# gnosisguild/stylus-zkvm-verifiers

Measured on AMD Instinct MI355X. Metric: Groth16 proofs verified/sec (BN254), higher is better.
Workload: dtype u32

## Files before the change

stylus_zkvm_verifiers_amd/build.py:

```python
import concurrent.futures as cf
import glob
import os
import subprocess
import sys

HERE = os.path.dirname(os.path.abspath(__file__))
CSRC = os.path.join(HERE, 'csrc')
BUILD = os.path.join(CSRC, 'build')
LIB = os.path.join(HERE, 'libzkv_mi355x.so')
UNITS = ['k_setup', 'k_gt', 'k_prep', 'k_msm', 'k_pair', 'k_wide', 'k_precompile', 'k_wire', 'k_mixed', 'k_diag', 'k_plonk', 'k_plonk_keys', 'k_plonk_set', 'k_pset_agg', 'k_agg', 'k_gset', 'k_gset_pair', 'k_gset_agg', 'k_gset_agg_pair', 'k_gateway', 'k_gateway_keys', 'k_risc0_router', 'k_setincl', 'k_rzrouter_set', 'k_wire_rzset', 'k_selftest', 'k_selftest_pair', 'zkv_capi']
FLAGS = ['--offload-arch=gfx950', '-O3', '-std=c++17', '-fPIC', '-fvisibility=hidden', '-DZKV_FP_MUL_NOINLINE',
         '-Rpass-analysis=kernel-resource-usage']
UNIT_FLAGS = {}
COMPILE_TIMEOUT_S = 1500
EXTRA = os.environ.get('ZKV_EXTRA_FLAGS', '').split()


def _hipcc():
    for c in ('/opt/rocm/bin/hipcc', 'hipcc'):
        if os.path.sep not in c or os.path.exists(c):
            return c
    return 'hipcc'


def _deps_mtime():
    files = glob.glob(os.path.join(CSRC, '*.h')) + [os.path.join(HERE, '..', 'include', f) for f in ('zkv.h', 'zkv_groth16_set.h', 'zkv_sp1_gateway.h', 'zkv_sp1_gateway_wire.h', 'zkv_sp1_gateway_keys.h', 'zkv_plonk_keys.h', 'zkv_plonk_set.h', 'zkv_plonk_set_agg.h', 'zkv_diag_primitive.h', 'zkv_diag_prep.h', 'zkv_diag_gt.h', 'zkv_risc0_set_inclusion.h', 'zkv_risc0_router.h', 'zkv_risc0_router_wire.h', 'zkv_risc0_router_set.h', 'zkv_risc0_router_set_wire.h')]
    return max(os.path.getmtime(f) for f in files)


def _compile(unit, force, dep_m):
    src = os.path.join(CSRC, unit + '.hip')
    obj = os.path.join(BUILD, unit + '.o')
    log = os.path.join(BUILD, unit + '.log')
    if not force and os.path.exists(obj) and os.path.getmtime(obj) >= max(os.path.getmtime(src), dep_m):
        return unit, 'cached'
    cmd = [_hipcc()] + FLAGS + UNIT_FLAGS.get(unit, []) + EXTRA + ['-c', src, '-o', obj]
    with open(log, 'w') as lf:
        try:
            rc = subprocess.run(cmd, stdout=lf, stderr=subprocess.STDOUT, timeout=COMPILE_TIMEOUT_S, cwd=CSRC).returncode
        except subprocess.TimeoutExpired:
            rc = 124
    if rc != 0:
        tail = open(log).read()[-4000:]
        raise RuntimeError('hipcc failed for %s (rc=%d)\n%s' % (unit, rc, tail))
    return unit, 'built'


def build(force=False, verbose=True):
    os.makedirs(BUILD, exist_ok=True)
    dep_m = _deps_mtime()
    with cf.ThreadPoolExecutor(max_workers=min(7, os.cpu_count() or 4)) as ex:
        results = list(ex.map(lambda u: _compile(u, force, dep_m), UNITS))
    objs = [os.path.join(BUILD, u + '.o') for u in UNITS]
    need_link = force or not os.path.exists(LIB) or any(os.path.getmtime(o) > os.path.getmtime(LIB) for o in objs)
    if need_link:
        subprocess.check_call([_hipcc(), '--offload-arch=gfx950', '-shared', '-fPIC', '-o', LIB] + objs)
    if verbose:
        print('libzkv_mi355x.so:', ', '.join('%s=%s' % r for r in results), '(linked)' if need_link else '(up to date)')
    return LIB
# ... 27 lines not shown
```

stylus_zkvm_verifiers_amd/csrc/k_pair.hip:

```cpp
#define ZKV_PAIRED 1
#include "zkv_internal.h"
#include "zkv_agg.h"

namespace zkv {

#ifndef ZKV_PAIR_WAVES
#define ZKV_PAIR_WAVES 1
#endif
constexpr int PAIR_BLOCK = ZKV_BLOCK * ZKV_PAIR_WAVES;

__device__ __forceinline__ Fp2 ld_b(const Workspace& ws, int word0, size_t i) {
    Fp2 r; r.h = ws_ld(ws.prep, ws.cap, word0 + 8 * (int)(threadIdx.x & 1u), i);
    return r;
}

__global__ __launch_bounds__(ZKV_BLOCK, 2) void k_g2chk2(size_t n, Workspace ws, uint8_t* __restrict__ status) {
    size_t i = ((size_t)blockIdx.x * ZKV_BLOCK + threadIdx.x) >> 1;
    if (i >= n) return;
    uint32_t flags = ws.flags[i];
    if (!(flags & FL_ALIVE) || (flags & FL_B_INF)) return;
    Fp2 bx = ld_b(ws, 32, i), by = ld_b(ws, 48, i);
    bool ok = g2_in_subgroup(bx, by);
    if (!ok && !(threadIdx.x & 1u)) { ws.g2bad[i] = 1; status[i] = ST_VERIFICATION_FAILED; }
}

#if defined(ZKV_STAMPS)
__device__ unsigned long long* g_zkv_stamps = nullptr;
extern "C" __attribute__((visibility("default"))) int zkv_diag_set_stamps(void* dev_ptr) {
    return (int)hipMemcpyToSymbol(HIP_SYMBOL(g_zkv_stamps), &dev_ptr, sizeof(dev_ptr));
}
__device__ __forceinline__ void zkv_stamp(unsigned kernel, unsigned slot) {
    if ((threadIdx.x & 63u) != 0 || !g_zkv_stamps) return;
    unsigned long long* row = g_zkv_stamps + ((size_t)kernel * gridDim.x * (blockDim.x >> 6) + (size_t)blockIdx.x * (blockDim.x >> 6) + (threadIdx.x >> 6)) * 8;
    row[slot] = __builtin_amdgcn_s_memrealtime();
    row[4 + slot] = __builtin_amdgcn_s_memtime();
    if (slot == 0) { row[2] = __builtin_amdgcn_s_getreg((31 << 11) | 4); row[3] = __builtin_amdgcn_s_getreg((31 << 11) | 20); }
}
#define ZKV_STAMP(k, s) zkv_stamp(k, s)
#else
#define ZKV_STAMP(k, s) ((void)0)
#endif

__global__ __launch_bounds__(PAIR_BLOCK, 2) void k_miller2(size_t n, const VkTables* __restrict__ vk, const uint32_t* __restrict__ mconst, Workspace ws, uint8_t* __restrict__ status) {
    __shared__ uint32_t lds[(48 + 24) * PAIR_BLOCK];
    ZKV_STAMP(0, 0);
    size_t i = ((size_t)blockIdx.x * PAIR_BLOCK + threadIdx.x) >> 1;
    if (i >= n) return;
    uint32_t flags = ws.flags[i];
    if (!(flags & FL_ALIVE)) return;
    const uint32_t par = threadIdx.x & 1u;
    uint32_t* wl = lds + (threadIdx.x >> 6) * ((48 + 24) * ZKV_BLOCK) + (threadIdx.x & 63u);
    LRef fm = l_ref(wl);
    LRef tm = l_ref(wl + 48 * ZKV_BLOCK);
    SoaRef norm = {ws.norm, ws.cap, (uint32_t)i * 4u};
    SoaRef bsrc = {ws.prep + 32 * ws.cap, ws.cap, (uint32_t)(8 * par * ws.cap + i) * 4u};
    const uint32_t* start = mconst ? mconst + 96 : nullptr;
    if (!miller_loop_p(vk, flags, norm, bsrc, fm, tm, true, start)) {
        if (!par) { ws.g2bad[i] = 1; status[i] = ST_VERIFICATION_FAILED; }
        return;
    }
    MRef out = m_ref(ws.f + (size_t)(8 * par) * ws.cap + i, (uint32_t)ws.cap, 16);
    if (start) f12m_copy(out, fm);
    else {
        MRef ab = m_ref((uint32_t*)vk->f_alpha_beta + 8 * par, 1, 16);
        f12m_mul_body(out, fm, ab, false);
    }
    ZKV_STAMP(0, 1);
}

__global__ __launch_bounds__(PAIR_BLOCK, 2) void k_finalexp2(size_t n, GtTab gt, long long gt_rel, long long gt_crel, Workspace ws, uint8_t* __restrict__ status) {
    __shared__ uint32_t lds[54 * PAIR_BLOCK];
    ZKV_STAMP(1, 0);
    size_t i = ((size_t)blockIdx.x * PAIR_BLOCK + threadIdx.x) >> 1;
    if (i >= n) return;
    uint32_t flags = ws.flags[i];
    if (!(flags & FL_ALIVE) || ws.g2bad[i]) return;
    const uint32_t par = threadIdx.x & 1u;
    uint32_t* wl = lds + (threadIdx.x >> 6) * (54 * ZKV_BLOCK) + (threadIdx.x & 63u);
    L9Ref acc = l9_ref(wl);
    const GtRef g = {gt.tab != nullptr, (ptrdiff_t)gt_rel, ws.prep + 64 * ws.cap, gt.nw[0], gt.nw[1], gt.cache ? ws.gtag : nullptr, (ptrdiff_t)gt_crel};
    bool one = final_exp_prog_p(ws.f, ws.fe, ws.cap, (uint32_t)(8 * par * ws.cap + i) * 4u, acc, g);
    if (!par) status[i] = one ? ST_OK : ST_VERIFICATION_FAILED;
    ZKV_STAMP(1, 1);
}

ZKV_HD bool pair_all(bool mine) {
    uint32_t v = mine ? 0u : 1u;
    v |= zkv_partner_u32(v);
    return v == 0;
}
// ... 270 lines not shown
```

stylus_zkvm_verifiers_amd/csrc/k_selftest_pair.hip:

```cpp
#define ZKV_PAIRED 1
#define ZKV_SELFTEST_BODIES 1
#include "zkv_internal.h"
#include "zkv_selftest.h"

namespace zkv {

__global__ __launch_bounds__(64) void k_selftest_pair(int op, int in_w, int out_w, const uint32_t* __restrict__ in, uint32_t* __restrict__ out) {
    __shared__ uint32_t lds[(144 + 54) * 64];
    const size_t i = (size_t)blockIdx.x * 32 + (threadIdx.x >> 1);
    selftest_pair(op, in + i * (size_t)in_w, out + i * (size_t)out_w, lds + threadIdx.x);
}
template <int S>
__device__ __forceinline__ void selftest_wide_body(int op, int in_w, int out_w, const uint32_t* in, uint32_t* out, uint32_t* lds) {
    constexpr int GROUP = 16 * S;
    const uint32_t g = threadIdx.x / GROUP;
    WL w;
    w.q = (int)((threadIdx.x >> 1) & 7u);
    if (w.q >= 6) w.q -= 6;
    w.s = (int)((threadIdx.x % GROUP) >> 4);
    const size_t i = (size_t)blockIdx.x * (64 / GROUP) + g;
    selftest_wide<S>(op, in + i * (size_t)in_w, out + i * (size_t)out_w, lds + g * ST_WIDE_SLOT, w);
}
__global__ __launch_bounds__(64) void k_selftest_wide_s1(int op, int in_w, int out_w, const uint32_t* __restrict__ in, uint32_t* __restrict__ out) {
    __shared__ uint32_t lds[4 * ST_WIDE_SLOT];
    selftest_wide_body<1>(op, in_w, out_w, in, out, lds);
}
__global__ __launch_bounds__(64) void k_selftest_wide_s4(int op, int in_w, int out_w, const uint32_t* __restrict__ in, uint32_t* __restrict__ out) {
    __shared__ uint32_t lds[ST_WIDE_SLOT];
    selftest_wide_body<4>(op, in_w, out_w, in, out, lds);
}

void launch_selftest_pair(int mapping, int op, unsigned waves, const uint32_t* in, uint32_t* out, hipStream_t s) {
    int iw = 0, ow = 0;
    selftest_io(mapping, op, &iw, &ow);
    if (mapping == 1) hipLaunchKernelGGL(k_selftest_pair, dim3(waves), dim3(64), 0, s, op, iw, ow, in, out);
    else if (mapping == 2) hipLaunchKernelGGL(k_selftest_wide_s1, dim3(waves), dim3(64), 0, s, op, iw, ow, in, out);
    else hipLaunchKernelGGL(k_selftest_wide_s4, dim3(waves), dim3(64), 0, s, op, iw, ow, in, out);
}

}
```

stylus_zkvm_verifiers_amd/csrc/zkv_capi.hip:

```cpp
#include <hip/hip_runtime.h>
#include <condition_variable>
#include <functional>
#include <memory>
#include <mutex>
#include <new>
#include <math.h>
#include <stdio.h>
#include <stdlib.h>
#include <string.h>
#include <system_error>
#include <thread>
#include <utility>
#include <vector>

#include "../../include/zkv.h"
#include "../../include/zkv_groth16_set.h"
#include "../../include/zkv_sp1_gateway.h"
#include "../../include/zkv_sp1_gateway_wire.h"
#include "../../include/zkv_sp1_gateway_keys.h"
#include "../../include/zkv_plonk_keys.h"
#include "../../include/zkv_plonk_set.h"
#include "../../include/zkv_plonk_set_agg.h"
#include "../../include/zkv_diag_primitive.h"
#include "../../include/zkv_diag_prep.h"
#include "../../include/zkv_diag_gt.h"
#include "../../include/zkv_risc0_set_inclusion.h"
#include "../../include/zkv_risc0_router.h"
#include "../../include/zkv_risc0_router_wire.h"
#include "../../include/zkv_risc0_router_set.h"
#include "../../include/zkv_risc0_router_set_wire.h"
#include "zkv_host_abi.h"
#include "zkv_host_vk.h"
#include "zkv_internal.h"
#include "zkv_devmem.h"
#include "zkv_plonk.h"
#include "zkv_agg.h"
#include "zkv_gset_layout.h"
#include "zkv_selftest.h"
#include "zkv_setincl.h"
#include "zkv_rzrouter_prep.h"
#include "zkv_wire_rzrouter.h"
#include "zkv_rzrouter_set.h"
#include "zkv_wire_rzset.h"
#include <sys/random.h>

using namespace zkv;

#define ZKV_EXPORT extern "C" __attribute__((visibility("default")))

struct ChunkMem {
    DevBuf<uint32_t> ws_prep, ws_norm, ws_f, ws_fe, ws_flags, ws_g2bad;
    DevBuf<uint8_t> ws_gtag;
    Workspace ws = {nullptr, nullptr, nullptr, nullptr, nullptr, nullptr, 0};
    DevBuf<uint8_t> d_a, d_b, d_status, d_recv;
    DevBuf<uint64_t> d_off, d_pvoff;
    DevBuf<uint32_t> d_inst_idx;
// ... 3386 lines not shown
    if (shader_clock_ghz) *shader_clock_ghz = clk[1] ? 0.1 * (double)clk[0] / (double)clk[1] : 0.0;
    return ZKV_OK;
}
ZKV_EXPORT int zkv_diag_mulmod_rate(int device, int kind, int waves_per_simd, uint32_t iters, double* mulmods_per_s, double* shader_clock_ghz) {
    if (kind < 0 || kind > 4 || waves_per_simd < 1 || waves_per_simd > 8 || !iters || !mulmods_per_s) return ZKV_ERR_INVALID_ARG;
    return run_diag(device, false, kind, waves_per_simd, iters, mulmods_per_s, shader_clock_ghz);
}
ZKV_EXPORT int zkv_diag_issue_rate(int device, int kind, int waves_per_simd, uint32_t iters, double* lane_instr_per_s, double* shader_clock_ghz) {
    if (kind < 0 || kind > 2 || waves_per_simd < 1 || waves_per_simd > 8 || !iters || !lane_instr_per_s) return ZKV_ERR_INVALID_ARG;
    return run_diag(device, true, kind, waves_per_simd, iters, lane_instr_per_s, shader_clock_ghz);
}

ZKV_EXPORT int zkv_diag_primitive(int device, int mapping, int op, size_t n, const uint32_t* in, uint32_t* out) {
    int iw = 0, ow = 0;
    if (!selftest_io(mapping, op, &iw, &ow) || n == 0 || n > ZKV_DIAG_PRIMITIVE_MAX_CASES || !in || !out) return ZKV_ERR_INVALID_ARG;
    int nd = 0;
    if (hipGetDeviceCount(&nd) != hipSuccess || nd <= 0) { (void)hipGetLastError(); return ZKV_ERR_NO_DEVICE; }
    if (device < 0 || device >= nd || !device_is_gfx950(device)) return ZKV_ERR_NO_DEVICE;
    HIP_TRY(hipSetDevice(device));
    const size_t per = (size_t)selftest_cases_per_wave(mapping), waves = (n + per - 1) / per, padded = waves * per;
    DevBuf<uint32_t> d_in, d_out;
    if (d_in.alloc(padded * (size_t)iw * 4) || d_out.alloc(padded * (size_t)ow * 4)) return ZKV_ERR_OOM;
    bool ok = hipMemset(d_in, 0, padded * (size_t)iw * 4) == hipSuccess && hipMemcpy(d_in, in, n * (size_t)iw * 4, hipMemcpyHostToDevice) == hipSuccess;
    if (ok) {
        if (mapping == 0) launch_selftest_lane(op, (unsigned)waves, d_in, d_out, nullptr);
        else launch_selftest_pair(mapping, op, (unsigned)waves, d_in, d_out, nullptr);
        ok = hipGetLastError() == hipSuccess && hipDeviceSynchronize() == hipSuccess &&
             hipMemcpy(out, d_out, n * (size_t)ow * 4, hipMemcpyDeviceToHost) == hipSuccess;
    }
    if (!ok) { (void)hipGetLastError(); return ZKV_ERR_HIP; }
    return ZKV_OK;
}

static_assert(ZKV_DIAG_PREP_SIGNALS == MAX_VAR, "zkv_diag_prep.h documents MAX_VAR signal rows");
ZKV_EXPORT int zkv_diag_prep_signals(zkv_ctx* c, size_t n, uint32_t* signals, uint32_t* flags) {
    if (!c || !signals || !flags || n == 0) return ZKV_ERR_INVALID_ARG;
    if (is_sharded(c) || (c->vm != ZKV_VM_RISC0 && c->vm != ZKV_VM_SP1) || c->agg_on) return ZKV_ERR_INVALID_ARG;
    int nd = 0;
    if (hipGetDeviceCount(&nd) != hipSuccess || nd <= 0) { (void)hipGetLastError(); return ZKV_ERR_NO_DEVICE; }
    if (c->device < 0 || c->device >= nd || !device_is_gfx950(c->device)) return ZKV_ERR_NO_DEVICE;
    std::lock_guard<std::mutex> lk(c->mu);
    if (!c->dev_ready || !c->ws.prep || n > c->last_chunk_n || n > c->ws.cap) return ZKV_ERR_INVALID_ARG;
    HIP_TRY(hipSetDevice(c->device));
    HIP_TRY(hipDeviceSynchronize());
    const size_t rows = (size_t)8 * MAX_VAR;
    std::vector<uint32_t> t(rows * n);
    HIP_TRY(hipMemcpy2D(t.data(), 4 * n, c->ws.prep + (size_t)64 * c->ws.cap, 4 * c->ws.cap, 4 * n, rows, hipMemcpyDeviceToHost));
    HIP_TRY(hipMemcpy(flags, c->ws.flags, 4 * n, hipMemcpyDeviceToHost));
    for (size_t j = 0; j < n; j++)
        for (size_t r = 0; r < rows; r++) signals[j * rows + r] = t[r * n + j];
    return ZKV_OK;
}

ZKV_EXPORT int zkv_ctx_vm(const zkv_ctx* c) { return c ? c->vm : ZKV_ERR_INVALID_ARG; }
ZKV_EXPORT int zkv_ctx_set_lanes_per_proof(zkv_ctx* c, int lanes) {
    if (!c || (lanes != 0 && lanes != 2 && lanes != 16 && lanes != 64 && lanes != 128)) return ZKV_ERR_INVALID_ARG;
    if (is_sharded(c)) { for (auto* k : c->shards) { const int rc = zkv_ctx_set_lanes_per_proof(k, lanes); if (rc != ZKV_OK) return rc; } return ZKV_OK; }
    if (c->vm == ZKV_VM_MIXED) {
        for (auto* k : c->kid) { const int rc = zkv_ctx_set_lanes_per_proof(k, lanes); if (rc != ZKV_OK) return rc; }
    }
    if (c->vm == ZKV_VM_RISC0_SETINCL) { const int rc = zkv_ctx_set_lanes_per_proof(c->kid[0], lanes); if (rc != ZKV_OK) return rc; }
    if (c->vm == ZKV_VM_RISC0_ROUTER && c->kid[0]) { const int rc = zkv_ctx_set_lanes_per_proof(c->kid[0], lanes); if (rc != ZKV_OK) return rc; }
    for (auto* k : c->gw_route) { if (!k) continue; const int rc = zkv_ctx_set_lanes_per_proof(k, lanes); if (rc != ZKV_OK) return rc; }
    if (c->gw_group) { const int rc = zkv_ctx_set_lanes_per_proof(c->gw_group, lanes); if (rc != ZKV_OK) return rc; }
    std::lock_guard<std::mutex> lk(c->mu);
    c->lanes = lanes;
// ... 906 lines not shown
```

stylus_zkvm_verifiers_amd/csrc/zkv_internal.h:

```cpp
#pragma once
#include <hip/hip_runtime.h>
#include "zkv_verify.h"

namespace zkv {

constexpr int WS_PREP_WORDS = 64 + 8 * MAX_VAR;
constexpr int WS_NORM_WORDS = 48;
constexpr int WS_F_WORDS = 96;
constexpr int WS_FE_WORDS = 7 * 96;
struct Workspace {
    uint32_t* prep; uint32_t* norm; uint32_t* f; uint32_t* fe; uint32_t* flags;
    uint32_t* g2bad;
    size_t cap;
    uint8_t* gtag;
};

constexpr int ZKV_BLOCK = 64;

__device__ __forceinline__ Fp ws_ld(const uint32_t* base, size_t cap, int word0, size_t i) {
    Fp r;
#pragma unroll
    for (int k = 0; k < 8; k++) r.v[k] = base[(size_t)(word0 + k) * cap + i];
    return r;
}
// ... 212 lines not shown
void launch_gset_agg_fprod(size_t n, size_t n2, uint32_t sub, uint32_t g, const Workspace& ws, const uint32_t* agg, const Workspace& ws2, const uint32_t* psl,
                           hipStream_t s);
void launch_gset_agg_mark(size_t n, uint32_t sub, uint32_t g, const Workspace& ws, const uint32_t* agg, const uint8_t* status2, const uint32_t* psl,
                          uint8_t* status, unsigned long long* counters, hipStream_t s);

#ifndef ZKV_PLONK_PROOF_BYTES
#define ZKV_PLONK_PROOF_BYTES 868
#endif
struct PlonkKeyRaw; struct PlonkKey;
void launch_plonk_setup(const PlonkKeyRaw* d_raw, PlonkKey* d_key, hipStream_t s);
void launch_plonk_setup_keys(const PlonkKeyRaw* d_raw, PlonkKey* d_key, hipStream_t s);
void launch_plonk_prep(const PrepArgs& a, const PlonkKey* d_key, const Workspace& ws, hipStream_t s);
void launch_plonk_prep_keys(const PrepArgs& a, const PlonkKey* d_key, const Workspace& ws, hipStream_t s);
struct PsetChunk {
    size_t m, slot0;
    const uint32_t* idx; const uint32_t* skey;
    const PlonkKey* keys; const uint32_t* ok;
    const uint8_t* proofs; uint32_t proof_stride;
    const uint8_t* inputs; uint32_t input_stride;
    uint32_t* plonk_tab;
    uint8_t* status;
};
void launch_pset_setup(uint32_t n_keys, const PlonkKeyRaw* d_raw, PlonkKey* d_keys, const VkTables* d_tabs, uint32_t* d_ok, hipStream_t s);
void launch_pset_prep(const PsetChunk& c, const Workspace& ws, hipStream_t s);
void launch_pset_agg_reduce(size_t m, uint32_t sub, const Workspace& ws, const uint32_t* agg, const Workspace& ws2, uint8_t* status2, const uint32_t* psl,
                            bool park, hipStream_t s);
void launch_pset_agg_combine(size_t n2, uint32_t wide, const Workspace& ws2, uint8_t* status2, const uint32_t* psl, hipStream_t s);

int read_wait_faults(unsigned long long* out);
void launch_diag_mulmod(int kind, unsigned blocks, uint32_t iters, uint32_t* out, unsigned long long* clk, hipStream_t s);
void launch_diag_issue(int kind, unsigned blocks, uint32_t iters, uint32_t* out, unsigned long long* clk, hipStream_t s);
void launch_selftest_lane(int op, unsigned waves, const uint32_t* in, uint32_t* out, hipStream_t s);
void launch_selftest_pair(int mapping, int op, unsigned waves, const uint32_t* in, uint32_t* out, hipStream_t s);

struct AggTables; struct AggSeed;
void launch_setup_agg(const VkRaw* d_raw, const VkTables* d_tab, AggTables* d_agg, hipStream_t s);
void launch_agg_g1(size_t n, const VkTables* d_tab, const InstTab* inst_tab, const Workspace& ws, uint32_t* agg, const AggSeed& seed, bool sums, hipStream_t s);
void launch_agg_reduce(size_t n, uint32_t sub, bool sums, uint32_t g, const VkTables* d_tab, const Workspace& ws, const uint32_t* agg, const AggTables* tab,
                       const Workspace& ws2, uint8_t* status2, bool park, hipStream_t s);
void launch_agg_combine(size_t n64, size_t n2, uint32_t wide, const AggTables* tab, const Workspace& ws2, uint8_t* status2, hipStream_t s);
void launch_agg_miller(size_t n, uint32_t g, const VkTables* d_tab, const Workspace& ws, uint8_t* status, hipStream_t s);
void launch_agg_fprod(size_t n, size_t n2, uint32_t sub, uint32_t g, const Workspace& ws, const uint32_t* agg, const Workspace& ws2, hipStream_t s);
void launch_agg_mark(size_t n, uint32_t sub, uint32_t g, const Workspace& ws, const uint32_t* agg, const uint8_t* status2, uint8_t* status, unsigned long long* counters,
                     uint32_t* idx, hipStream_t s);
void launch_agg_gather(size_t n, const Workspace& ws, const uint32_t* agg, const unsigned long long* counters, const uint32_t* idx, const Workspace& ws3,
                       uint8_t* status3, hipStream_t s);
void launch_agg_plonk_g1(size_t n, const Workspace& ws, uint32_t* agg, const AggSeed& seed, hipStream_t s);
void launch_agg_plonk_norm(size_t n, const Workspace& ws, const uint32_t* agg, const unsigned long long* counters, const uint32_t* idx, const Workspace& ws3,
                           uint8_t* status3, hipStream_t s);
void launch_agg_scatter(size_t n, const unsigned long long* counters, const uint32_t* idx, const uint8_t* status3, uint8_t* status, hipStream_t s);

void launch_ecadd(size_t n, const uint8_t* in, uint8_t* out, uint8_t* ok, hipStream_t s);
void launch_ecmul(size_t n, const uint8_t* in, uint8_t* out, uint8_t* ok, hipStream_t s);
void launch_pairing(size_t n, uint32_t k, const uint8_t* in, const Workspace& ws, uint8_t* result, uint8_t* ok, hipStream_t s);
uint32_t pairing_group(uint32_t k);
void launch_pairing_w(size_t n, uint32_t k, const uint8_t* in, const Workspace& ws, uint8_t* result, uint8_t* ok, hipStream_t s);

}
```

stylus_zkvm_verifiers_amd/csrc/zkv_selftest.h:

```cpp
#pragma once
#include <stdint.h>

namespace zkv {

inline bool selftest_io(int mapping, int op, int* in_w, int* out_w) {
    static const int LANE[11][2] = {{24, 128}, {24, 16}, {16, 16}, {8, 8}, {32, 64}, {24, 40}, {8, 12}, {64, 72}, {32, 2}, {128, 248}, {112, 384}};
    static const int PAIR[10][2] = {{32, 80}, {162, 18}, {36, 18}, {240, 11 * 96}, {96, 2 * 96}, {32, 4}, {192, 6}, {80, 2}, {192, 816}, {32, 4}};
    static const int WIDE[4][2] = {{240, 8 * 96}, {96, 96}, {96, 16}, {288, 0}};
    const int* w = nullptr;
    if (mapping == 0 && op >= 0 && op < 11) w = LANE[op];
    else if (mapping == 1 && op >= 0 && op < 10) w = PAIR[op];
    else if ((mapping == 2 || mapping == 3) && op >= 0 && op < 4) w = WIDE[op];
    if (!w) return false;
    *in_w = w[0]; *out_w = (mapping == 3 && op == 2) ? 4 * w[1] : w[1];
    if (mapping >= 2 && op == 3) *out_w = 2 * (48 + 48 * 8 * (mapping == 3 ? 4 : 1)) + 5 * 96 + 48;
    return true;
}
inline int selftest_cases_per_wave(int mapping) { return mapping == 0 ? 64 : mapping == 1 ? 32 : mapping == 2 ? 4 : 1; }

}

#if defined(ZKV_SELFTEST_BODIES)
#if defined(ZKV_PAIRED)
#include "zkv_tower_wide.h"
// ... 217 lines not shown
                line_add(T, qx, qy, l0, l1, l3);
            }
            m_st_f2(tm, 0, T.x); m_st_f2(tm, 1, T.y); m_st_f2(tm, 2, T.z);
        };
        auto put = [&](uint32_t* o, const Fp2& l0, const Fp2& l1, const Fp2& l3) {
            for (int k = 0; k < 3; k++) st_st(o + 16 * k + 8 * par, m_ld_f2(tm, k).h);
            st_st(o + 48 + 8 * par, l0.h); st_st(o + 64 + 8 * par, l1.h); st_st(o + 80 + 8 * par, l3.h);
        };
        Fp2 l0, l1, l3, t0, t1, t3;
        load_t(); step(0, t0, t1, t3); put(out, t0, t1, t3);
        for (int kind = 1; kind <= 4; kind++) { load_t(); step(kind, l0, l1, l3); put(out + 96 * kind, l0, l1, l3); }
        f12m_copy(fm, m_ref((uint32_t*)in + 96 + 8 * par, 1, 16));
        {
            const Fp2 c3 = f2_mul_fp(t1, norm.fp(0)), c4 = f2_mul_fp(t3, norm.fp(8));
            f12m_mul_by_034_body(fm, t0, c3, c4);
        }
        f12m_copy(m_ref(out + 480 + 8 * par, 1, 16), fm);
        load_t(); step(0, l0, l1, l3); step(1, l0, l1, l3); step(0, l0, l1, l3);
        for (int k = 0; k < 3; k++) st_st(out + 576 + 16 * k + 8 * par, m_ld_f2(tm, k).h);
        load_t(); g2m_line_dbl(tm, &l0, &l1, &l3); put(out + 624, l0, l1, l3);
        const Fp2 qx = st_ldh(in + 48, par), qy = st_ldh(in + 64, par);
        load_t(); g2m_line_add(tm, &qx, &qy, &l0, &l1, &l3); put(out + 720, l0, l1, l3);
        break;
    }
    case 9: {
        const Fp2 qx = st_ldh(in, par), qy = st_ldh(in + 16, par);
        out[par] = g2_on_twist(qx, qy) ? 1u : 0u; out[2 + par] = g2_in_subgroup(qx, qy) ? 1u : 0u;
        break;
    }
    default: break;
    }
}

constexpr int ST_WIDE_SLOT = 96 + 48 + 13 * 16 + W_RED_WORDS;
template <int S> ZKV_HD int st_group_lane(WL w, uint32_t par) {
#if defined(__HIP_DEVICE_COMPILE__)
    (void)w; (void)par;
    return (int)(__builtin_amdgcn_mbcnt_hi(~0u, __builtin_amdgcn_mbcnt_lo(~0u, 0u)) & (uint32_t)(16 * S - 1));
#else
    return 16 * w.s + 2 * w.q + (int)par;
#endif
}
template <int S> ZKV_HD void selftest_wide(int op, const uint32_t* in, uint32_t* out, uint32_t* g, WL w) {
    const uint32_t par = zkv_parity();
    const int q = w.q;
    uint32_t* base = g + 8 * par;
    const MRef A = m_ref(base, 1, 16), B = m_ref(base + 96, 1, 16), D = m_ref(base + 192, 1, 16), red = m_ref(base + 288, 1, 16);
    const MRef ga = m_ref((uint32_t*)in + 8 * par, 1, 16), gb = m_ref((uint32_t*)in + 96 + 8 * par, 1, 16);
    auto put = [&](int k) { w12_copy(m_ref(out + 96 * k + 8 * par, 1, 16), D, q); };
    switch (op) {
    case 0: {
        const Fp2 c0 = st_ldh(in + 192, par), c3 = st_ldh(in + 208, par), c4 = st_ldh(in + 224, par);
        w12_copy(A, ga, q); w12_copy(B, gb, q);
        w12_copy(D, A, q); w12_mul<S>(D, D, B, w, false, red); put(0);
        w12_copy(D, A, q); w12_mul<S>(D, D, B, w, true, red); put(1);
        w12_copy(D, A, q); w12_sqr<S>(D, w, red); put(2);
        w12_copy(D, A, q); w12_mul_sparse<S>(D, &c0, &c3, &c4, w, false, red); put(3);
        w12_copy(D, A, q); w12_mul_sparse<S>(D, &c3, &c3, &c4, w, true, red); put(4);
        for (int k = 1; k <= 3; k++) { w12_frob(D, A, k, q); put(4 + k); }
        break;
    }
    case 1: {
        w12_copy(D, ga, q); w12_cyclo_sqr<S>(D, w, red); put(0);
        break;
    }
    case 2: {
// ... 50 lines not shown
```

stylus_zkvm_verifiers_amd/csrc/zkv_verify.h:

```cpp
#pragma once
#include "zkv_tower_mem.h"
#include "zkv_sha256.h"
#include "zkv_gt.h"

namespace zkv {

enum : uint8_t {
    ST_OK = 0, ST_VERIFICATION_FAILED = 1, ST_INVALID_INITIALIZATION = 2, ST_ALREADY_INITIALIZED = 3,
    ST_INVALID_PROOF_DATA = 4, ST_SELECTOR_MISMATCH = 5,
    ST_BAD_CALLDATA = 6
};
enum : uint32_t { FL_ALIVE = 1u, FL_A_INF = 2u, FL_B_INF = 4u, FL_C_INF = 8u, FL_L_INF = 16u };

constexpr int N_LINES = 88;
constexpr int MSM_MAX_WINDOWS = 32;
constexpr int MSM_DIGITS = 256;
constexpr int MAX_IC = 6;
constexpr int MAX_VAR = 5;

struct VkRaw {
    uint32_t alpha[2][8];
    uint32_t beta[4][8], gamma[4][8], delta[4][8];
    uint32_t ic[MAX_IC][2][8];
    uint32_t n_ic;
    uint32_t fixed_scalar[MAX_IC][8];
    uint32_t is_fixed[MAX_IC];
    uint32_t n_var;
    uint32_t var_ic[MAX_VAR];
    uint32_t var_windows[MAX_VAR];
};

struct VkTables {
    G1A base; uint32_t base_inf; uint32_t n_var; uint32_t var_windows[MAX_VAR];
    uint32_t vk_valid;
// ... 228 lines not shown
            }
            if (do_l) fixed_line_mul(fm, lines0[li], n.lxs, n.lys);
            if (do_c) fixed_line_mul(fm, lines1[li], n.cxs, n.cys);
            li++;
        }
    }
    Fp2 qx[2], qy[2];
    g2_frob_affine(qx[0], qy[0], bx, by);
    g2_frob2_affine(qx[1], qy[1], bx, by);
    qy[1] = f2_neg(qy[1]);
#pragma unroll 1
    for (int s = 0; s < 2; s++) {
        if (do_t) {
            g2m_line_add(tm, &qx[s], &qy[s], &l0, &l1, &l3);
            if (do_ab) var_line_mul(fm, l0, l1, l3, n.axs, n.ays);
        }
        if (do_l) fixed_line_mul(fm, lines0[li], n.lxs, n.lys);
        if (do_c) fixed_line_mul(fm, lines1[li], n.cxs, n.cys);
        li++;
    }
    return !(check_b && do_t) || miller_point_closes(tm, bx, by);
}

#if defined(ZKV_PAIRED)
struct SoaRef {
    const uint32_t* p; size_t stride; uint32_t off;
    ZKV_HD Fp fp(int word0) const {
        Fp r;
#pragma unroll
        for (int k = 0; k < 8; k++) r.v[k] = *(const uint32_t*)((const char*)(p + (size_t)(word0 + k) * stride) + off);
        return r;
    }
};
template <class RF, class RT>
ZKV_HD bool miller_loop_p(const VkTables* vkp, uint32_t flags, SoaRef norm, SoaRef bsrc, RF fm, RT tm, bool check_b = false, const uint32_t* start = nullptr) {
    const uint8_t KIND[ZKV_MILLER_STEPS] = ZKV_MILLER_STEP_KIND;
    const bool with_fixed = vkp != nullptr;
    const bool do_ab = !(flags & (FL_A_INF | FL_B_INF));
    const bool do_t = do_ab || (check_b && !(flags & FL_B_INF));
    const bool do_l = with_fixed && !(flags & FL_L_INF) && !vkp->skip_fixed[0], do_c = with_fixed && !(flags & FL_C_INF) && !vkp->skip_fixed[1];
    if (start) f12m_copy(fm, m_ref(const_cast<uint32_t*>(start) + 8 * zkv_parity(), 1, 16));
    else f12m_set_one(fm);
    { Fp2 bx, by; bx.h = bsrc.fp(0); by.h = bsrc.fp(16); m_st_f2(tm, 0, bx); m_st_f2(tm, 1, by); m_st_f2(tm, 2, f2_one()); }
    const uint32_t slot = zkv_wave_slot_parity();
#pragma unroll 1
    for (int li = 0; li < ZKV_MILLER_STEPS; li++) {
        const int kind = KIND[li];
        zkv_fair_share(slot);
#if defined(__HIP_DEVICE_COMPILE__)
        asm volatile("" : "+v"(norm.off), "+v"(bsrc.off));
#endif
        if (kind == 0 && li != 0) { ZKV_MARK("begin sqr"); f12m_sqr_body(fm); ZKV_MARK("end sqr"); }
        if (do_t) {
            Fp2 l0, l1, l3;
            G2H T; T.x = m_ld_f2(tm, 0); T.y = m_ld_f2(tm, 1); T.z = m_ld_f2(tm, 2);
            if (kind == 0) { ZKV_MARK("begin linedbl"); line_dbl(T, l0, l1, l3); ZKV_MARK("end linedbl"); }
            else {
                Fp2 qx, qy; qx.h = bsrc.fp(0); qy.h = bsrc.fp(16);
                if (kind == 2) qy = f2_neg(qy);
                else if (kind == 3) { Fp2 x, y; g2_frob_affine(x, y, qx, qy); qx = x; qy = y; }
                else if (kind == 4) { Fp2 x, y; g2_frob2_affine(x, y, qx, qy); qx = x; qy = f2_neg(y); }
                ZKV_MARK("begin lineadd"); line_add(T, qx, qy, l0, l1, l3); ZKV_MARK("end lineadd");
            }
            m_st_f2(tm, 0, T.x); m_st_f2(tm, 1, T.y); m_st_f2(tm, 2, T.z);
            if (do_ab) {
                ZKV_MARK("begin mul034");
                const Fp2 c3 = f2_mul_fp(l1, norm.fp(0)), c4 = f2_mul_fp(l3, norm.fp(8));
                f12m_mul_by_034_body(fm, l0, c3, c4);
                ZKV_MARK("end mul034");
            }
        }
#pragma unroll 1
        for (int j = 0; j < 2; j++) {
            if (j == 0 ? !do_l : !do_c) continue;
            ZKV_MARK("begin mul134");
            const LineAffC& L = vkp->lines[j][li];
            const Fp2 c3 = f2_mul_fp(f2_const(L.nl), norm.fp(16 + 16 * j)), c4 = f2_mul_fp(f2_const(L.c), norm.fp(24 + 16 * j));
            f12m_mul_by_134_body(fm, c3, c4);
            ZKV_MARK("end mul134");
        }
    }
    if (!check_b || !do_t) return true;
    Fp2 qx, qy; qx.h = bsrc.fp(0); qy.h = bsrc.fp(16);
    return miller_point_closes(tm, qx, qy);
}
template <int G, class RF>
// ... 432 lines not shown
```

Baseline: 7.102 million.

## Compute Miller-loop line steps with lazy-reduced limb sums and folded scaling

Adds new line doubling and addition routines that work on unreduced 29-bit limb column sums. They fold the G1-point scaling of the line coefficients into the line computation and update the G2 accumulator in place, instead of forming l1 and l3 and then multiplying by the normalised coordinates. The production Miller kernel switches to this path through a template flag. A self-test kernel and a diagnostic C API are added to check the new steps. The intent is to cut the full modular reductions per step, at the cost of more delicate limb-bound reasoning and possible register pressure.

```diff
diff --git a/include/zkv_diag_line_steps.h b/include/zkv_diag_line_steps.h
--- /dev/null
+++ b/include/zkv_diag_line_steps.h
@@ -0,0 +1,17 @@
+#ifndef ZKV_DIAG_LINE_STEPS_H
+#define ZKV_DIAG_LINE_STEPS_H
+#include "zkv_diag_primitive.h"
+
+#ifdef __cplusplus
+extern "C" {
+#endif
+
+#define ZKV_DIAG_LINE_STEPS_IN 192
+#define ZKV_DIAG_LINE_STEPS_OUT 624
+
+int zkv_diag_line_steps(int device, size_t n, const uint32_t* in, uint32_t* out);
+
+#ifdef __cplusplus
+}
+#endif
+#endif
diff --git a/stylus_zkvm_verifiers_amd/build.py b/stylus_zkvm_verifiers_amd/build.py
--- a/stylus_zkvm_verifiers_amd/build.py
+++ b/stylus_zkvm_verifiers_amd/build.py
@@ -24,7 +24,7 @@
 
 
 def _deps_mtime():
-    files = glob.glob(os.path.join(CSRC, '*.h')) + [os.path.join(HERE, '..', 'include', f) for f in ('zkv.h', 'zkv_groth16_set.h', 'zkv_sp1_gateway.h', 'zkv_sp1_gateway_wire.h', 'zkv_sp1_gateway_keys.h', 'zkv_plonk_keys.h', 'zkv_plonk_set.h', 'zkv_plonk_set_agg.h', 'zkv_diag_primitive.h', 'zkv_diag_prep.h', 'zkv_diag_gt.h', 'zkv_risc0_set_inclusion.h', 'zkv_risc0_router.h', 'zkv_risc0_router_wire.h', 'zkv_risc0_router_set.h', 'zkv_risc0_router_set_wire.h')]
+    files = glob.glob(os.path.join(CSRC, '*.h')) + [os.path.join(HERE, '..', 'include', f) for f in ('zkv.h', 'zkv_groth16_set.h', 'zkv_sp1_gateway.h', 'zkv_sp1_gateway_wire.h', 'zkv_sp1_gateway_keys.h', 'zkv_plonk_keys.h', 'zkv_plonk_set.h', 'zkv_plonk_set_agg.h', 'zkv_diag_primitive.h', 'zkv_diag_line_steps.h', 'zkv_diag_prep.h', 'zkv_diag_gt.h', 'zkv_risc0_set_inclusion.h', 'zkv_risc0_router.h', 'zkv_risc0_router_wire.h', 'zkv_risc0_router_set.h', 'zkv_risc0_router_set_wire.h')]
     return max(os.path.getmtime(f) for f in files)
 
 
diff --git a/stylus_zkvm_verifiers_amd/csrc/k_pair.hip b/stylus_zkvm_verifiers_amd/csrc/k_pair.hip
--- a/stylus_zkvm_verifiers_amd/csrc/k_pair.hip
+++ b/stylus_zkvm_verifiers_amd/csrc/k_pair.hip
@@ -55,7 +55,7 @@
     SoaRef norm = {ws.norm, ws.cap, (uint32_t)i * 4u};
     SoaRef bsrc = {ws.prep + 32 * ws.cap, ws.cap, (uint32_t)(8 * par * ws.cap + i) * 4u};
     const uint32_t* start = mconst ? mconst + 96 : nullptr;
-    if (!miller_loop_p(vk, flags, norm, bsrc, fm, tm, true, start)) {
+    if (!miller_loop_p<true>(vk, flags, norm, bsrc, fm, tm, true, start)) {
         if (!par) { ws.g2bad[i] = 1; status[i] = ST_VERIFICATION_FAILED; }
         return;
     }
diff --git a/stylus_zkvm_verifiers_amd/csrc/k_selftest_pair.hip b/stylus_zkvm_verifiers_amd/csrc/k_selftest_pair.hip
--- a/stylus_zkvm_verifiers_amd/csrc/k_selftest_pair.hip
+++ b/stylus_zkvm_verifiers_amd/csrc/k_selftest_pair.hip
@@ -9,6 +9,11 @@
     __shared__ uint32_t lds[(144 + 54) * 64];
     const size_t i = (size_t)blockIdx.x * 32 + (threadIdx.x >> 1);
     selftest_pair(op, in + i * (size_t)in_w, out + i * (size_t)out_w, lds + threadIdx.x);
+}
+__global__ __launch_bounds__(64) void k_selftest_line_sums(const uint32_t* __restrict__ in, uint32_t* __restrict__ out) {
+    __shared__ uint32_t lds[(48 + 24) * 64];
+    const size_t i = (size_t)blockIdx.x * 32 + (threadIdx.x >> 1);
+    selftest_line_sums(in + i * (size_t)ST_LINE_SUMS_IN, out + i * (size_t)ST_LINE_SUMS_OUT, lds + threadIdx.x);
 }
 template <int S>
 __device__ __forceinline__ void selftest_wide_body(int op, int in_w, int out_w, const uint32_t* in, uint32_t* out, uint32_t* lds) {
@@ -37,5 +42,8 @@
     else if (mapping == 2) hipLaunchKernelGGL(k_selftest_wide_s1, dim3(waves), dim3(64), 0, s, op, iw, ow, in, out);
     else hipLaunchKernelGGL(k_selftest_wide_s4, dim3(waves), dim3(64), 0, s, op, iw, ow, in, out);
 }
+void launch_selftest_line_sums(unsigned waves, const uint32_t* in, uint32_t* out, hipStream_t s) {
+    hipLaunchKernelGGL(k_selftest_line_sums, dim3(waves), dim3(64), 0, s, in, out);
+}
 
 }
diff --git a/stylus_zkvm_verifiers_amd/csrc/zkv_capi.hip b/stylus_zkvm_verifiers_amd/csrc/zkv_capi.hip
--- a/stylus_zkvm_verifiers_amd/csrc/zkv_capi.hip
+++ b/stylus_zkvm_verifiers_amd/csrc/zkv_capi.hip
@@ -22,6 +22,7 @@
 #include "../../include/zkv_plonk_set.h"
 #include "../../include/zkv_plonk_set_agg.h"
 #include "../../include/zkv_diag_primitive.h"
+#include "../../include/zkv_diag_line_steps.h"
 #include "../../include/zkv_diag_prep.h"
 #include "../../include/zkv_diag_gt.h"
 #include "../../include/zkv_risc0_set_inclusion.h"
@@ -3474,6 +3475,26 @@
     return ZKV_OK;
 }
 
+static_assert(ZKV_DIAG_LINE_STEPS_IN == 192 && ZKV_DIAG_LINE_STEPS_OUT == 624, "zkv_diag_line_steps.h documents the rows of selftest_line_sums");
+ZKV_EXPORT int zkv_diag_line_steps(int device, size_t n, const uint32_t* in, uint32_t* out) {
+    if (n == 0 || n > ZKV_DIAG_PRIMITIVE_MAX_CASES || !in || !out) return ZKV_ERR_INVALID_ARG;
+    int nd = 0;
+    if (hipGetDeviceCount(&nd) != hipSuccess || nd <= 0) { (void)hipGetLastError(); return ZKV_ERR_NO_DEVICE; }
+    if (device < 0 || device >= nd || !device_is_gfx950(device)) return ZKV_ERR_NO_DEVICE;
+    HIP_TRY(hipSetDevice(device));
+    const size_t iw = ZKV_DIAG_LINE_STEPS_IN, ow = ZKV_DIAG_LINE_STEPS_OUT, waves = (n + 31) / 32, padded = waves * 32;
+    DevBuf<uint32_t> d_in, d_out;
+    if (d_in.alloc(padded * iw * 4) || d_out.alloc(padded * ow * 4)) return ZKV_ERR_OOM;
+    bool ok = hipMemset(d_in, 0, padded * iw * 4) == hipSuccess && hipMemcpy(d_in, in, n * iw * 4, hipMemcpyHostToDevice) == hipSuccess;
+    if (ok) {
+        launch_selftest_line_sums((unsigned)waves, d_in, d_out, nullptr);
+        ok = hipGetLastError() == hipSuccess && hipDeviceSynchronize() == hipSuccess &&
+             hipMemcpy(out, d_out, n * ow * 4, hipMemcpyDeviceToHost) == hipSuccess;
+    }
+    if (!ok) { (void)hipGetLastError(); return ZKV_ERR_HIP; }
+    return ZKV_OK;
+}
+
 static_assert(ZKV_DIAG_PREP_SIGNALS == MAX_VAR, "zkv_diag_prep.h documents MAX_VAR signal rows");
 ZKV_EXPORT int zkv_diag_prep_signals(zkv_ctx* c, size_t n, uint32_t* signals, uint32_t* flags) {
     if (!c || !signals || !flags || n == 0) return ZKV_ERR_INVALID_ARG;
diff --git a/stylus_zkvm_verifiers_amd/csrc/zkv_internal.h b/stylus_zkvm_verifiers_amd/csrc/zkv_internal.h
--- a/stylus_zkvm_verifiers_amd/csrc/zkv_internal.h
+++ b/stylus_zkvm_verifiers_amd/csrc/zkv_internal.h
@@ -268,6 +268,7 @@
 void launch_diag_issue(int kind, unsigned blocks, uint32_t iters, uint32_t* out, unsigned long long* clk, hipStream_t s);
 void launch_selftest_lane(int op, unsigned waves, const uint32_t* in, uint32_t* out, hipStream_t s);
 void launch_selftest_pair(int mapping, int op, unsigned waves, const uint32_t* in, uint32_t* out, hipStream_t s);
+void launch_selftest_line_sums(unsigned waves, const uint32_t* in, uint32_t* out, hipStream_t s);
 
 struct AggTables; struct AggSeed;
 void launch_setup_agg(const VkRaw* d_raw, const VkTables* d_tab, AggTables* d_agg, hipStream_t s);
diff --git a/stylus_zkvm_verifiers_amd/csrc/zkv_line_sums.h b/stylus_zkvm_verifiers_amd/csrc/zkv_line_sums.h
--- /dev/null
+++ b/stylus_zkvm_verifiers_amd/csrc/zkv_line_sums.h
@@ -0,0 +1,255 @@
+#pragma once
+#include "zkv_tower_mem.h"
+
+#if defined(ZKV_PAIRED)
+#if defined(ZKV_COUNT_FP_MUL)
+static thread_local long long zkv_line_mad_excess_counter = 0;
+#endif
+
+namespace zkv {
+
+ZKV_HD void limbs_partner(const uint32_t (&a)[9], uint32_t (&p)[9]) {
+#pragma unroll
+    for (int i = 0; i < 9; i++) p[i] = zkv_partner_u32(a[i]);
+}
+ZKV_HD void limbs_carry(uint32_t (&a)[9]) {
+#pragma unroll
+    for (int k = 0; k < 8; k++) { a[k + 1] += a[k] >> 29; a[k] &= 0x1fffffffu; }
+}
+ZKV_HD void limbs_carry_signed(uint32_t (&a)[9]) {
+#pragma unroll
+    for (int k = 0; k < 8; k++) { a[k + 1] += (uint32_t)((int32_t)a[k] >> 29); a[k] &= 0x1fffffffu; }
+}
+ZKV_HD void limbs_carry_x3(uint32_t (&a)[9]) {
+    ZKV_COUNT_MADS_ISSUED(8);
+    uint32_t c = 0;
+#pragma unroll
+    for (int k = 0; k < 8; k++) { const uint64_t t = (uint64_t)a[k] * 3u + c; a[k] = (uint32_t)t & 0x1fffffffu; c = (uint32_t)(t >> 29); }
+    a[8] = a[8] * 3u + c;
+}
+template <int K, int LIFT> ZKV_HD void limbs_kp_fat(uint32_t (&F)[9]) {
+    const uint32_t P29[9] = ZKV_FP_P29_LIMBS;
+#pragma unroll
+    for (int i = 0; i < 9; i++) F[i] = (uint32_t)K * P29[i];
+    limbs_carry(F);
+#pragma unroll
+    for (int i = 0; i < 9; i++) F[i] += (i < 8 ? (uint32_t)LIFT << 29 : 0u) - (i > 0 ? (uint32_t)LIFT : 0u);
+}
+template <bool SIGNED> ZKV_HD void limbs_half_carry(uint32_t (&a)[9]) {
+    const uint32_t P29[9] = ZKV_FP_P29_LIMBS;
+    const uint32_t m = 0u - (a[0] & 1u);
+#pragma unroll
+    for (int i = 0; i < 9; i++) a[i] += P29[i] & m;
+    if (SIGNED) limbs_carry_signed(a);
+    else limbs_carry(a);
+#pragma unroll
+    for (int k = 0; k < 8; k++) a[k] = (a[k] >> 1) | ((a[k + 1] & 1u) << 28);
+    a[8] >>= 1;
+}
+ZKV_HD void limbs_y(const uint32_t (&y)[9], uint32_t (&U)[9], uint32_t (&V)[9]) {
+    const uint32_t FAT[9] = ZKV_FP_FAT8P_LIMBS;
+    const bool even = zkv_parity() == 0;
+#pragma unroll
+    for (int i = 0; i < 9; i++) { U[i] = zkv_pair_even_u32(y[i]); const uint32_t v = zkv_pair_odd_u32(y[i]); V[i] = even ? FAT[i] - v : v; }
+}
+ZKV_HD void limbs_y_neg(const uint32_t (&y)[9], uint32_t (&U)[9], uint32_t (&V)[9]) {
+    const uint32_t FAT[9] = ZKV_FP_FAT8P_LIMBS;
+    const bool even = zkv_parity() == 0;
+#pragma unroll
+    for (int i = 0; i < 9; i++) { U[i] = FAT[i] - zkv_pair_even_u32(y[i]); const uint32_t v = zkv_pair_odd_u32(y[i]); V[i] = even ? v : FAT[i] - v; }
+}
+ZKV_HD void f2_sum_cross_neg(uint64_t (&col)[18], const uint32_t (&ao)[9], const uint32_t (&ap)[9], const uint32_t (&nU)[9], const uint32_t (&nV)[9]) {
+#if defined(ZKV_COUNT_FP_MUL)
+    zkv_fp_mul_counter += 2;
+#endif
+    ZKV_LIMBS_BELOW(ao, 29); ZKV_LIMBS_BELOW(ap, 29); ZKV_LIMBS_BELOW(nU, 30); ZKV_LIMBS_BELOW(nV, 30);
+    fp_mac81(col, ao, nU); fp_mac81(col, ap, nV);
+}
+ZKV_HD void fp_sum_scale(uint64_t (&col)[18], const uint32_t (&a)[9], const uint32_t (&k)[9]) {
+#if defined(ZKV_COUNT_FP_MUL)
+    zkv_fp_mul_counter += 1;
+#endif
+    ZKV_LIMBS_BELOW(a, 31); ZKV_LIMBS_BELOW(k, 29);
+    fp_mac81(col, a, k);
+}
+ZKV_HD void f2_sum_close_limbs(uint64_t (&col)[18], uint32_t (&r)[9]) {
+    fp_reduce_cols_limbs(col, r);
+#if defined(__HIP_DEVICE_COMPILE__)
+    limbs_pin(r);
+    __builtin_amdgcn_sched_barrier(0);
+#endif
+}
+ZKV_HD void limbs_sqr_factors_5p(const uint32_t (&own)[9], const uint32_t (&par)[9], uint32_t (&M)[9], uint32_t (&N)[9]) {
+    uint32_t F[9]; limbs_kp_fat<5, 1>(F);
+    const bool odd = zkv_parity() != 0;
+#pragma unroll
+    for (int i = 0; i < 9; i++) {
+        M[i] = par[i] + (odd ? par[i] : own[i]);
+        N[i] = own[i] + (odd ? 0u : F[i] - par[i]);
+    }
+    limbs_carry(N);
+}
+ZKV_HD void limbs_sqr_factors_neg3(const uint32_t (&own)[9], const uint32_t (&par)[9], uint32_t (&M)[9], uint32_t (&N)[9]) {
+    uint32_t F[9]; limbs_kp_fat<2, 1>(F);
+    const bool odd = zkv_parity() != 0;
+#pragma unroll
+    for (int i = 0; i < 9; i++) {
+        M[i] = par[i] + (odd ? par[i] : own[i]);
+        N[i] = F[i] - own[i] + (odd ? 0u : par[i]);
+    }
+    limbs_carry_x3(N);
+}
+
+#if defined(ZKV_COUNT_FP_MUL)
+struct LineCharge {
+    unsigned long long c0, i0, m0;
+    LineCharge() : c0(zkv_mad_counter), i0(zkv_mad_issued_counter), m0(zkv_fp_mul_counter) {}
+    void settle(unsigned long long mads, unsigned long long muls) {
+        zkv_line_mad_excess_counter += (long long)(zkv_mad_issued_counter - i0) - (long long)mads;
+        zkv_mad_counter = c0 + mads; zkv_mad_issued_counter = i0 + mads; zkv_fp_mul_counter = m0 + muls;
+    }
+};
+#endif
+
+template <class RT, class SC> ZKV_HD void line_dbl_sums(RT tm, Fp2& l0, Fp2& c3, Fp2& c4, SC scale) {
+#if defined(ZKV_COUNT_FP_MUL)
+    LineCharge charge;
+#endif
+    const uint32_t FAT[9] = ZKV_FP_FAT8P_LIMBS;
+    const Fp2C b3c = ZKV_TWIST_3B;
+    uint64_t col[18];
+    uint32_t yo[9], yp[9], tU[9], tV[9], M[9], N[9], xo[9], xp[9];
+    uint32_t b[9], h[9], m[9], e[9], q[9], qp[9], k9[9];
+    f2_limbs_x(m_ld_f2(tm, 1).h, yo, yp);
+    f2_limbs_sqr(yo, yp, M, N);
+    f2_sum_open(col); f2_sum_sqr(col, M, N); f2_sum_close_limbs(col, b);
+    fp_unpack29(m_ld_f2(tm, 2).h, xo);
+    limbs_y(xo, tU, tV);
+#pragma unroll
+    for (int i = 0; i < 9; i++) { q[i] = yo[i] << 1; qp[i] = yp[i] << 1; }
+    f2_sum_open(col); f2_sum_cross_dbl(col, q, qp, tU, tV); f2_sum_close_limbs(col, h);
+    { Fp2 hp; hp.h = fp_pack29(h); l0 = f2_neg(hp); }
+    limbs_partner(xo, xp);
+    f2_limbs_sqr(xo, xp, M, N);
+    f2_sum_open(col); f2_sum_sqr(col, M, N); f2_sum_close_limbs(col, q);
+    limbs_partner(q, qp);
+    {
+        uint32_t em = zkv_parity() == 0 ? ~0u : 0u;
+#if defined(__HIP_DEVICE_COMPILE__)
+        asm volatile("" : "+v"(em));
+#endif
+        uint32_t y1[9]; fp_unpack29(b3c.c0, tU); fp_unpack29(b3c.c1, y1);
+#pragma unroll
+        for (int i = 0; i < 9; i++) tV[i] = y1[i] + (em & (FAT[i] - 2u * y1[i]));
+    }
+    f2_sum_open(col); f2_sum_cross(col, q, qp, tU, tV); f2_sum_close_limbs(col, e);
+    f2_limbs_x(m_ld_f2(tm, 0).h, xo, xp);
+    limbs_y(yo, tU, tV);
+    f2_sum_open(col); f2_sum_cross(col, xo, xp, tU, tV); f2_sum_close_limbs(col, m);
+    {
+        const bool odd = zkv_parity() != 0;
+#pragma unroll
+        for (int i = 0; i < 9; i++) { M[i] = xp[i] + (odd ? xp[i] : xo[i]); N[i] = xo[i] + (odd ? 0u : FAT[i] - xp[i]); }
+        limbs_carry_x3(N);
+    }
+    f2_sum_open(col); f2_sum_sqr(col, M, N); f2_sum_close_limbs(col, q);
+    fp_unpack29(scale(0), k9);
+    f2_sum_open(col); fp_sum_scale(col, q, k9); c3.h = f2_sum_close(col);
+#pragma unroll
+    for (int i = 0; i < 9; i++) q[i] = e[i] + FAT[i] - b[i];
+    fp_unpack29(scale(1), k9);
+    f2_sum_open(col); fp_sum_scale(col, q, k9); c4.h = f2_sum_close(col);
+#pragma unroll
+    for (int i = 0; i < 9; i++) q[i] = b[i] + FAT[i] - 3u * e[i];
+    limbs_half_carry<true>(q);
+    limbs_partner(q, qp);
+    limbs_y(m, tU, tV);
+    f2_sum_open(col); f2_sum_cross(col, q, qp, tU, tV);
+    { Fp2 o; o.h = f2_sum_close(col); m_st_f2(tm, 0, o); }
+#pragma unroll
+    for (int i = 0; i < 9; i++) q[i] = b[i] + 3u * e[i];
+    limbs_half_carry<false>(q);
+    limbs_partner(q, qp);
+    limbs_sqr_factors_5p(q, qp, M, N);
+    f2_sum_open(col); f2_sum_sqr(col, M, N);
+    limbs_partner(e, qp);
+    limbs_sqr_factors_neg3(e, qp, M, N);
+    f2_sum_sqr(col, M, N);
+    { Fp2 o; o.h = f2_sum_close(col); m_st_f2(tm, 1, o); }
+    limbs_partner(b, qp);
+    limbs_y(h, tU, tV);
+    f2_sum_open(col); f2_sum_cross(col, b, qp, tU, tV);
+    { Fp2 o; o.h = f2_sum_close(col); m_st_f2(tm, 2, o); }
+#if defined(ZKV_COUNT_FP_MUL)
+    charge.settle(4 * 243 + 6 * 162 + 2 * 162, 4 * 2 + 6 + 2);
+#endif
+}
+
+template <class RT, class SC> ZKV_HD void line_add_sums(RT tm, const Fp2& qx, const Fp2& qy, Fp2& l0, Fp2& c3, Fp2& c4, SC scale) {
+#if defined(ZKV_COUNT_FP_MUL)
+    LineCharge charge;
+#endif
+    const uint32_t FAT[9] = ZKV_FP_FAT8P_LIMBS;
+    uint32_t F4[9]; limbs_kp_fat<4, 2>(F4);
+    uint64_t col[18];
+    uint32_t zU[9], zV[9], ao[9], ap[9], bo[9], bp[9], tU[9], tV[9], M[9], N[9];
+    uint32_t th[9], la[9], e[9], f[9], g[9], w[9], k9[9];
+    f2_limbs_y(m_ld_f2(tm, 2).h, zU, zV);
+    f2_limbs_x(qx.h, ao, ap);
+    f2_sum_open(col); f2_sum_cross(col, ao, ap, zU, zV);
+    { Fp2 s; s.h = f2_sum_close(col); l0 = f2_sub(m_ld_f2(tm, 0), s); }
+    f2_limbs_x(qy.h, bo, bp);
+    f2_sum_open(col); f2_sum_cross(col, bo, bp, zU, zV);
+    { Fp2 s; s.h = f2_sum_close(col); s = f2_sub(m_ld_f2(tm, 1), s); fp_unpack29(s.h, th); }
+    fp_unpack29(l0.h, la);
+    limbs_y(th, tU, tV);
+    f2_sum_open(col); f2_sum_cross(col, ao, ap, tU, tV);
+    limbs_y_neg(la, tU, tV);
+    f2_sum_cross_neg(col, bo, bp, tU, tV); f2_sum_close_limbs(col, w);
+    fp_unpack29(scale(1), k9);
+    f2_sum_open(col); fp_sum_scale(col, w, k9); c4.h = f2_sum_close(col);
+#pragma unroll
+    for (int i = 0; i < 9; i++) w[i] = FAT[i] - th[i];
+    fp_unpack29(scale(0), k9);
+    f2_sum_open(col); fp_sum_scale(col, w, k9); c3.h = f2_sum_close(col);
+    limbs_partner(la, ap);
+    f2_limbs_sqr(la, ap, M, N);
+    f2_sum_open(col); f2_sum_sqr(col, M, N); f2_sum_close_limbs(col, ao);
+    limbs_partner(ao, ap);
+    limbs_y(la, tU, tV);
+    f2_sum_open(col); f2_sum_cross(col, ao, ap, tU, tV); f2_sum_close_limbs(col, e);
+    f2_limbs_y(m_ld_f2_again(tm, 0).h, tU, tV);
+    f2_sum_open(col); f2_sum_cross(col, ao, ap, tU, tV); f2_sum_close_limbs(col, g);
+    limbs_partner(th, bp);
+    f2_limbs_sqr(th, bp, M, N);
+    f2_sum_open(col); f2_sum_sqr(col, M, N); f2_sum_close_limbs(col, bo);
+    limbs_partner(bo, bp);
+    f2_sum_open(col); f2_sum_cross(col, bo, bp, zU, zV); f2_sum_close_limbs(col, f);
+#pragma unroll
+    for (int i = 0; i < 9; i++) w[i] = e[i] + f[i] + F4[i] - 2u * g[i];
+    limbs_carry(w);
+    limbs_partner(w, ap);
+    limbs_pin(la);
+    limbs_y(la, tU, tV);
+    f2_sum_open(col); f2_sum_cross(col, w, ap, tU, tV);
+    { Fp2 o; o.h = f2_sum_close(col); m_st_f2(tm, 0, o); }
+#pragma unroll
+    for (int i = 0; i < 9; i++) w[i] = 3u * g[i] + F4[i] - e[i] - f[i];
+    limbs_carry(w);
+    limbs_partner(w, ap);
+    limbs_pin(th);
+    limbs_y(th, tU, tV);
+    f2_sum_open(col); f2_sum_cross(col, w, ap, tU, tV);
+    { uint32_t y[9]; fp_unpack29(m_ld_f2_again(tm, 1).h, y); limbs_y_neg(y, tU, tV); }
+    limbs_partner(e, bp);
+    f2_sum_cross_neg(col, e, bp, tU, tV);
+    { Fp2 o; o.h = f2_sum_close(col); m_st_f2(tm, 1, o); }
+    f2_sum_open(col); f2_sum_cross(col, e, bp, zU, zV);
+    { Fp2 o; o.h = f2_sum_close(col); m_st_f2(tm, 2, o); }
+#if defined(ZKV_COUNT_FP_MUL)
+    charge.settle(11 * 243 + 2 * 162 + 2 * 162, 11 * 2 + 2 + 2);
+#endif
+}
+
+}
+#endif
diff --git a/stylus_zkvm_verifiers_amd/csrc/zkv_selftest.h b/stylus_zkvm_verifiers_amd/csrc/zkv_selftest.h
--- a/stylus_zkvm_verifiers_amd/csrc/zkv_selftest.h
+++ b/stylus_zkvm_verifiers_amd/csrc/zkv_selftest.h
@@ -273,6 +273,39 @@
     }
 }
 
+constexpr int ST_LINE_SUMS_IN = 192, ST_LINE_SUMS_OUT = 624;
+ZKV_HD void selftest_line_sums(const uint32_t* in, uint32_t* out, uint32_t* lds) {
+    const uint32_t par = zkv_parity();
+    const LRef fm = l_ref(lds), tm = l_ref(lds + 48 * 64);
+    SoaRef bsrc; bsrc.p = in + 48; bsrc.stride = 1; bsrc.off = 32u * par;
+    SoaRef norm; norm.p = in + 80; norm.stride = 1; norm.off = 0;
+    const auto scale = [&](int k) { return norm.fp(8 * k); };
+    auto load_t = [&]() { for (int k = 0; k < 3; k++) m_st_f2(tm, k, st_ldh(in + 16 * k, par)); };
+    auto step = [&](int kind, Fp2& l0, Fp2& c3, Fp2& c4) {
+        if (kind == 0) line_dbl_sums(tm, l0, c3, c4, scale);
+        else {
+            Fp2 qx, qy; qx.h = bsrc.fp(0); qy.h = bsrc.fp(16);
+            if (kind == 2) qy = f2_neg(qy);
+            else if (kind == 3) { Fp2 x, y; g2_frob_affine(x, y, qx, qy); qx = x; qy = y; }
+            else if (kind == 4) { Fp2 x, y; g2_frob2_affine(x, y, qx, qy); qx = x; qy = f2_neg(y); }
+            line_add_sums(tm, qx, qy, l0, c3, c4, scale);
+        }
+    };
+    auto put = [&](uint32_t* o, const Fp2& l0, const Fp2& c3, const Fp2& c4) {
+        for (int k = 0; k < 3; k++) st_st(o + 16 * k + 8 * par, m_ld_f2(tm, k).h);
+        st_st(o + 48 + 8 * par, l0.h); st_st(o + 64 + 8 * par, c3.h); st_st(o + 80 + 8 * par, c4.h);
+    };
+    Fp2 l0, c3, c4, t0, t3, t4;
+    load_t(); step(0, t0, t3, t4); put(out, t0, t3, t4);
+#pragma unroll 1
+    for (int kind = 1; kind <= 4; kind++) { load_t(); step(kind, l0, c3, c4); put(out + 96 * kind, l0, c3, c4); }
+    f12m_copy(fm, m_ref((uint32_t*)in + 96 + 8 * par, 1, 16));
+    f12m_mul_by_034_body(fm, t0, t3, t4);
+    f12m_copy(m_ref(out + 480 + 8 * par, 1, 16), fm);
+    load_t(); step(0, l0, c3, c4); step(1, l0, c3, c4); step(0, l0, c3, c4);
+    for (int k = 0; k < 3; k++) st_st(out + 576 + 16 * k + 8 * par, m_ld_f2(tm, k).h);
+}
+
 constexpr int ST_WIDE_SLOT = 96 + 48 + 13 * 16 + W_RED_WORDS;
 template <int S> ZKV_HD int st_group_lane(WL w, uint32_t par) {
 #if defined(__HIP_DEVICE_COMPILE__)
diff --git a/stylus_zkvm_verifiers_amd/csrc/zkv_verify.h b/stylus_zkvm_verifiers_amd/csrc/zkv_verify.h
--- a/stylus_zkvm_verifiers_amd/csrc/zkv_verify.h
+++ b/stylus_zkvm_verifiers_amd/csrc/zkv_verify.h
@@ -1,5 +1,6 @@
 #pragma once
 #include "zkv_tower_mem.h"
+#include "zkv_line_sums.h"
 #include "zkv_sha256.h"
 #include "zkv_gt.h"
 
@@ -294,7 +295,7 @@
         return r;
     }
 };
-template <class RF, class RT>
+template <bool LINE_SUMS = false, class RF, class RT>
 ZKV_HD bool miller_loop_p(const VkTables* vkp, uint32_t flags, SoaRef norm, SoaRef bsrc, RF fm, RT tm, bool check_b = false, const uint32_t* start = nullptr) {
     const uint8_t KIND[ZKV_MILLER_STEPS] = ZKV_MILLER_STEP_KIND;
     const bool with_fixed = vkp != nullptr;
@@ -313,7 +314,20 @@
         asm volatile("" : "+v"(norm.off), "+v"(bsrc.off));
 #endif
         if (kind == 0 && li != 0) { ZKV_MARK("begin sqr"); f12m_sqr_body(fm); ZKV_MARK("end sqr"); }
-        if (do_t) {
+        if (LINE_SUMS && do_t) {
+            Fp2 l0, c3, c4;
+            const auto scale = [&](int k) { return norm.fp(8 * k); };
+            if (kind == 0) { ZKV_MARK("begin linedbl"); line_dbl_sums(tm, l0, c3, c4, scale); ZKV_MARK("end linedbl"); }
+            else {
+                Fp2 qx, qy; qx.h = bsrc.fp(0); qy.h = bsrc.fp(16);
+                if (kind == 2) qy = f2_neg(qy);
+                else if (kind == 3) { Fp2 x, y; g2_frob_affine(x, y, qx, qy); qx = x; qy = y; }
+                else if (kind == 4) { Fp2 x, y; g2_frob2_affine(x, y, qx, qy); qx = x; qy = f2_neg(y); }
+                ZKV_MARK("begin lineadd"); line_add_sums(tm, qx, qy, l0, c3, c4, scale); ZKV_MARK("end lineadd");
+            }
+            if (do_ab) { ZKV_MARK("begin mul034"); f12m_mul_by_034_body(fm, l0, c3, c4); ZKV_MARK("end mul034"); }
+        }
+        if (!LINE_SUMS && do_t) {
             Fp2 l0, l1, l3;
             G2H T; T.x = m_ld_f2(tm, 0); T.y = m_ld_f2(tm, 1); T.z = m_ld_f2(tm, 2);
             if (kind == 0) { ZKV_MARK("begin linedbl"); line_dbl(T, l0, l1, l3); ZKV_MARK("end linedbl"); }
diff --git a/stylus_zkvm_verifiers_amd/diag_line_steps.py b/stylus_zkvm_verifiers_amd/diag_line_steps.py
--- /dev/null
+++ b/stylus_zkvm_verifiers_amd/diag_line_steps.py
@@ -0,0 +1,23 @@
+import ctypes as C
+
+from . import _lib
+
+IN_WORDS, OUT_WORDS = 192, 624
+
+SYMBOLS = {
+    'zkv_diag_line_steps': (C.c_int, [C.c_int, C.c_size_t, C.POINTER(C.c_uint32), C.POINTER(C.c_uint32)]),
+}
+
+_bound = None
+
+
+def lib():
+    global _bound
+    L = _lib.lib()
+    if _bound is not L:
+        for name, (res, args) in SYMBOLS.items():
+            fn = getattr(L, name)
+            fn.restype = res
+            fn.argtypes = args
+        _bound = L
+    return L
```

Measured after the change: 7.266 million, median of 6. 2.3% higher.
